# geometryxyz/mental-poker

Measured on AMD Instinct MI355X. Metric: shuffle proofs/sec (prove+verify), higher is better.
Workload: dtype u32 limbs (256-bit Montgomery: 9x29-bit lazy base field, 8x32 scalar field); 1 GPU; pairs: 52-card deck, m=2 n=26, stark curve, shuffle_and_remask + verify_shuffle; rccl_world=1, fixed_base_window_bits=21, unit_counted=prove+verify pairs, streams=1, aggregate_keys=1, transcript_lanes=1, prover_streams=1, pipeline_depth=0, validated_once=False, full=False

## Files before the change

### mental-poker_amd/csrc/engine_core.hpp

```cpp
#pragma once
#include "engine_base.hpp"
#include "kernels_bucket.hpp"
#include "kernels_canonical.hpp"
#include "kernels_sigma.hpp"
#include "kernels_open.hpp"
#include "kernels_deal.hpp"
#include "kernels_sample.hpp"
#include "kernels_screen.hpp"
#include "serialize_host.hpp"
#include "setup_host.hpp"

namespace mp {

static const uint32_t FCHUNK = 8;
static const uint32_t VCHUNK = 64;
static const uint32_t NORM_CHUNK = 64;
static const uint32_t BUCKET_MIN = 2048;
static const uint32_t BUCKET_MIN_SMALL_BATCH = 512;

struct PhaseDev {
  DevBuf<Term> recode, tables, fterms, vterms, cterms, cterms2, cterms0;
  DevBuf<Job> fjobs, vjobs, cjobs, cjobs2, cjobs0;
  DevBuf<BJob> bjobs;
  DevBuf<Term> bterms;
// ... 270 lines not shown
  Workspace ws;
  bool merged_verify = true;
  void set_merged_verify(bool on) override { merged_verify = on; }
  bool subgroup_check = !Cofactor<C>::ONE;
  void set_subgroup_check(bool on) override { subgroup_check = on && !Cofactor<C>::ONE; }
  void check_subgroup(Workspace& w, uint32_t B, uint32_t first, uint32_t count) {
    if (!subgroup_check || !count) return;
    SubgroupArgs a{w.P.p, w.status.p, w.Bpad, first};
    MP_RUN(k_subgroup_check, C, B, count, a);
  }
  void check_verify_inputs(Workspace& w, uint32_t B, const VerifyLay& l, bool keyed) {
    if (!validated) {
      check_subgroup(w, B, 0, l.pk + (keyed ? 1u : 0u));
      return;
    }
    if (!(validated & MP_VALIDATED_DECKS)) check_subgroup(w, B, l.deck, 2 * N);
    if (!(validated & MP_VALIDATED_SHUFFLED)) check_subgroup(w, B, l.shuf, 2 * N);
    const uint32_t rest = std::max(l.deck, l.shuf) + 2 * N;
    if (!(validated & MP_VALIDATED_PROOFS)) check_subgroup(w, B, rest, l.pk - rest);
    if (keyed) check_subgroup(w, B, l.pk, 1);
  }
  Workspace dws;
  void validate_decks_dev(size_t count, const uint8_t* decks, int32_t* status) override {
    rt::Stream s = ctx->stream;
    const uint32_t B = (uint32_t)count;
    Workspace& w = dws;
    w.fw = G_::FW;
    w.ensure(B, 1, 2 * N, 8, 0, 0, nwin, 4, s, 0);
    rt::dzero(w.status.p, (size_t)w.Bpad * 4, s);
    LoadPointsArgs a{decks, w.P.p, w.status.p, w.Bpad, 2 * N, 0};
    MP_RUN(k_load_points, C, B, 2 * N, a);
    if (!Cofactor<C>::ONE) {
      SubgroupArgs sa{w.P.p, w.status.p, w.Bpad, 0};
      MP_RUN(k_subgroup_check, C, B, 2 * N, sa);
    }
    rt::d2d(status, w.status.p, (size_t)B * 4, s);
    rt::stream_sync(s);
  }
  DevBuf<uint32_t> vflag;
  uint32_t* flag_word(bool vlane, rt::Stream s) {
    if (!vflag.n) vflag.alloc(2, s);
    rt::dzero(vflag.p + (vlane ? 1 : 0), 4, s);
    return vflag.p + (vlane ? 1 : 0);
  }
  bool read_flag(bool vlane) {
    uint32_t flag = 0;
    rt::d2h(&flag, vflag.p + (vlane ? 1 : 0), 4, ctx->stream);
    rt::stream_sync(ctx->stream);
    return flag != 0;
  }
  uint32_t nwin = 0;
  FbGeom fbg{8, 32, 255};
  uint32_t init_seed[8];
  DevBuf<uint8_t> io_a, io_b, io_c, io_d, io_e, io_f;
  DevBuf<int32_t> io_status;

  static bool wire_point_host(const uint8_t* p, Aff<C>& out) {
    alignas(8) uint8_t tmp[G_::PB];
    memcpy(tmp, p, G_::PB);
    return wire_to_aff<C>(tmp, out);
  }

  void build_plans(PlanSet* set, bool keyed) {
    rt::Stream s = ctx->stream;
    for (int k = 0; k < N_PLANS; ++k) {
      PlanSet& q = set[k];
      const PlanParams& pp = pprm[k];
      const uint32_t bmin = (bucket_min && k == 3) ? std::min(bucket_min, BUCKET_MIN_SMALL_BATCH) : bucket_min;
      const uint32_t pbits = bucket_bits_of(4 * N + 11 * m + 9);
      q.pplan = make_prove_plan(m, n, pp.fch, pp.vch, G_::PB, keyed, bmin, bk_windows(R::BITS, pbits), toom_cook && (k == 0 || k == 2 || k == 4), pp.vsp, pbits);
      q.vplan = make_verify_plan(m, n, pp.fch, pp.vch, G_::PB, keyed, bmin, bk_windows(R::BITS, pbits), pp.vsp, pbits);
      q.table_group = pp.grp;
      q.norm_chunk = pp.nch;
      for (int i = 0; i < 6; ++i) q.pph[i].upload(q.pplan.ph[i], s);
      q.vph.upload(q.vplan.ph, s);
      q.vmph.upload(q.vplan.mph, s);
      q.mjobs.upload(q.vplan.mjobs, s);
      q.mpairs.upload(q.vplan.mpairs, s);
      q.draws.upload(q.pplan.draws, s);
      q.lin.upload(q.pplan.lin, s);
      q.lin_src.upload(q.pplan.lin_src, s);
      q.lin_coef.upload(q.pplan.lin_coef, s);
      q.consts.upload(toom_constants(q.pplan.toom), s);
      q.pwire.upload(q.pplan.wire, s);
      q.vwire.upload(q.vplan.wire, s);
    }
  }
  void ensure_keyed() {
    if (psk_ready) return;
    build_plans(psk, true);
    const ProveLay& l = psk[0].pplan.lay;
    key_d_first = key_t_first = 0;
    for (int k = 0; k < N_PLANS; ++k)
      for (int i = 0; i < 6; ++i) {
        key_d_first = std::max(key_d_first, psk[k].pplan.ph[i].n_dslots);
        key_t_first = std::max(key_t_first, psk[k].pplan.ph[i].n_tslots);
      }
    std::vector<Term> rec, tab;
    for (uint32_t i = 0; i < N; ++i) rec.push_back(Term{l.rho + i, key_d_first + i});
    for (uint32_t w = 0; w < nwin; ++w) tab.push_back(Term{l.kw + w, key_t_first + w});
    key_recode.upload(rec, ctx->stream);
    key_tables.upload(tab, ctx->stream);
    psk_ready = true;
  }

  int init(mp_ctx* c, uint32_t m_, uint32_t n_, const uint8_t* params, const uint8_t* pk, uint32_t fb_bits, const mp_table* fb_from = nullptr) {
// ... 6 lines not shown
    point_bytes = G_::PB;
    if (G_::FW > 8) bucket_split_bits = 11;
    set_latency_batch(std::max<size_t>(40, (size_t)2560 * 52 / N));
    nwin = (uint32_t)vb_windows(R::BITS);
    default_plan_params();
    FixedBases fb{n};
    std::vector<Aff<C>> bases(fb.count());
    bool ok = true;
    Aff<C> G, H, gen, pkp;
    ok &= wire_point_host(params, G);
    for (uint32_t j = 0; j < n; ++j) ok &= wire_point_host(params + G_::PB * (1 + j), bases[fb.ck(j)]);
    ok &= wire_point_host(params + G_::PB * (1 + n), H);
    ok &= wire_point_host(params + G_::PB * (2 + n), gen);
    ok &= wire_point_host(pk, pkp);
    if (!ok) return fail(MP_ERR_BAD_ENCODING, "parameters / shared key: bad point encoding");
    ok = aff_in_subgroup_host<C>(G) && aff_in_subgroup_host<C>(H) && aff_in_subgroup_host<C>(gen) && aff_in_subgroup_host<C>(pkp);
    for (uint32_t j = 0; j < n; ++j) ok = ok && aff_in_subgroup_host<C>(bases[fb.ck(j)]);
    if (!ok) return fail(MP_ERR_BAD_ENCODING, "parameters / shared key: a point is not in the prime-order subgroup");
    bases[fb.H()] = H; bases[fb.G()] = G; bases[fb.pk()] = pkp; bases[fb.gen()] = gen;
    Jac<C> gs = jac_inf<C>();
    for (uint32_t j = 0; j < n; ++j) gs = jac_madd<C>(gs, bases[fb.ck(j)]);
    if (jac_is_inf<C>(gs)) {
      bases[fb.gsum()] = aff_inf<C>();
    } else {
      bases[fb.gsum()] = jac_to_aff_with_zinv<C>(gs, fe_inv<F>(gs.Z));
    }
    for (uint32_t i = 0; i < fb.count(); ++i)
      if (i != fb.gsum() && aff_is_inf<C>(bases[i])) return fail(MP_ERR_BAD_ENCODING, "parameters: a base is the point at infinity");

    rt::Stream s = ctx->stream;
    std::vector<uint32_t> flat(fb.count() * G_::PW);
    for (uint32_t i = 0; i < fb.count(); ++i) {
      fe_pack<F>(bases[i].x, &flat[i * G_::PW]);
      fe_pack<F>(bases[i].y, &flat[i * G_::PW + G_::FW]);
    }
    fbpts.upload(flat, s);
    if (fb_from) {
      if (fb_from->fb_bits != fb_bits || fb_from->n != n || fb_from->point_bytes != point_bytes || fb_from->ctx->device != ctx->device)
        return fail(MP_ERR_INTERNAL, "shared fixed-base tables: geometry or device mismatch");
      FB.borrow(fb_from->fixed_tables());
    } else {
      build_fixed_tables(fb.count());
    }

    build_plans(ps, false);
    {
      Blake2sState st;
      blake2s_init(st);
      uint32_t mblk[16] = {0};
      memcpy(mblk, "Shuffle Proof", 13);
      blake2s_compress(st, mblk, 13, true);
      memcpy(init_seed, st.h, 32);
    }
    rt::stream_sync(s);
    return MP_OK;
  }

  void normalize_flat(const uint32_t* src, uint32_t* dst, uint32_t* scratch, size_t count) {
    if (!count) return;
    const uint32_t ch = cur_norm_chunk;
    NormArgs a{src, dst, scratch, (uint32_t)count, (uint32_t)((count + ch - 1) / ch), ch};
    MP_RUN(k_normalize, C, a.nthreads, 1, a);
  }

  void build_narrow_tables(const uint32_t* pts, uint32_t nb, const FbGeom& gh, uint32_t h2, uint32_t* out) {
    rt::Stream s = ctx->stream;
    DevBuf<uint32_t> WJ, W, EJ, scratch;
    const size_t nwinpts = (size_t)nb * gh.windows, nent = nwinpts * gh.entries;
    WJ.alloc(nwinpts * G_::JW, s);
    W.alloc(nwinpts * G_::PW, s);
    EJ.alloc(nent * G_::JW, s);
    scratch.alloc(nent * G_::FW, s);
    FbWinArgs wa{pts, WJ.p, gh, h2};
    MP_RUN(k_fb_windows, C, nb, 1, wa);
    normalize_flat(WJ.p, W.p, scratch.p, nwinpts);
    FbFillArgs fa{W.p, EJ.p, gh};
    MP_RUN(k_fb_fill, C, (uint32_t)nwinpts, 1, fa);
    normalize_flat(EJ.p, out, scratch.p, nent);
    rt::stream_sync(s);
  }
  void build_fixed_tables(uint32_t nb) {
    rt::Stream s = ctx->stream;
    const uint32_t h = fbg.bits == 8 ? 8u : (fbg.bits + 1u) / 2u, h2 = fbg.bits == 8 ? 8u : fbg.bits - h;
    const FbGeom gh{h, fbg.bits == 8 ? fbg.windows : 2u * fbg.windows, (1u << h) - 1u};
    DevBuf<uint32_t> Th;
    Th.alloc((size_t)nb * gh.windows * gh.entries * G_::PW, s);
    build_narrow_tables(fbpts.p, nb, gh, h2, Th.p);
    if (fbg.bits == h) {
      std::swap(FB.p, Th.p);
      std::swap(FB.n, Th.n);
      return;
    }
    const size_t nentw = (size_t)nb * fbg.windows * fbg.entries;
    if (nentw >= ((size_t)1 << 32)) throw std::runtime_error("fixed-base table too large for one launch: use narrower windows");
    DevBuf<uint32_t> EJw, scratchw;
    EJw.alloc(nentw * G_::JW, s, false);
    scratchw.alloc(nentw * G_::FW, s, false);
    FB.alloc(nentw * G_::PW, s, false);
    FbWidenArgs ww{Th.p, EJw.p, gh, fbg};
    MP_RUN(k_fb_widen, C, (uint32_t)nentw, 1, ww);
    const size_t per = (size_t)1 << 26;
    for (size_t off = 0; off < nentw; off += per) {
      const size_t cnt = std::min(per, nentw - off);
      normalize_flat(EJw.p + off * G_::JW, FB.p + off * G_::PW, scratchw.p + off * G_::FW, cnt);
    }
    rt::stream_sync(s);
// ... 245 lines not shown
      CombineArgs a{w.J.p, w.P.p, ph.cjobs.p, ph.cterms.p, w.Bpad};
      run_combine(a, B, ph.n_c);
    }
    if (ph.n_c2) {
      CombineArgs a{w.J.p, w.P.p, ph.cjobs2.p, ph.cterms2.p, w.Bpad};
      run_combine(a, B, ph.n_c2);
    }
  }
  void run_normalize(PhaseDev& ph, Workspace& w, uint32_t B, uint32_t norm_only, uint32_t norm_skip, uint32_t* scratch) {
    std::vector<std::pair<uint32_t, uint32_t>> ranges;
    for (auto& r : ph.normalize)
      if ((norm_only == NO_SLOT || r.first == norm_only) && r.first != norm_skip) ranges.push_back(r);
    for (size_t i = 0; i < ranges.size();) {
      const size_t nr = std::min<size_t>(NORM_MAX_RANGES, ranges.size() - i);
      size_t last_elem = 0;
      for (size_t k = 0; k < nr; ++k)
        last_elem = std::max(last_elem, ((size_t)ranges[i + k].first + ranges[i + k].second) * w.Bpad);
      if (nr == 1 || last_elem >= ((size_t)1 << 32)) {
        auto& r = ranges[i];
        normalize_flat(w.J.p + j_off<C>(r.first, w.Bpad, 0), w.P.p + p_off<C>(r.first, w.Bpad, 0), scratch, (size_t)r.second * w.Bpad);
        ++i;
        continue;
      }
      NormMultiArgs a{};
      a.J = w.J.p; a.P = w.P.p; a.scratch = scratch;
      a.nr = (uint32_t)nr; a.chunk = cur_norm_chunk;
      uint32_t threads = 0, selem = 0;
      for (size_t k = 0; k < nr; ++k) {
        auto& r = ranges[i + k];
        const uint32_t cnt = r.second * w.Bpad;
        a.first[k] = r.first * w.Bpad;
        a.count[k] = cnt;
        a.tstart[k] = threads;
        a.sstart[k] = selem;
        threads += (cnt + cur_norm_chunk - 1) / cur_norm_chunk;
        selem += cnt;
      }
      a.tstart[nr] = threads;
      MP_RUN(k_normalize_multi, C, threads, 1, a);
      i += nr;
    }
  }

  FsStatementArgs statement_args(Workspace& w, uint32_t p_deck, uint32_t p_shuf, uint32_t p_cA, uint32_t s_x, uint32_t p_pk = NO_SLOT) {
    FsStatementArgs a{};
    a.f = FsDev{w.stage.p, w.seed.p, w.Bpad};
    a.S = w.S.p;
    a.P = w.P.p;
    a.fbpts = fbpts.p;
    memcpy(a.init_seed, init_seed, 32);
    a.m = m; a.n = n; a.N = N;
    a.p_deck = p_deck; a.p_shuf = p_shuf; a.p_cA = p_cA; a.s_x = s_x;
    a.p_pk = p_pk;
    a.W = nullptr;
    a.w_deck = a.w_shuf = NO_SLOT;
    return a;
  }
  FsqGeom fsq_geom(uint32_t B) const {
    uint32_t lpp = 64;
    while (lpp > 4 && (uint64_t)B * lpp > 65536u) lpp >>= 1;
    return FsqGeom{lpp, B};
  }
  static uint32_t fsq_waves(const FsqGeom& g) { return (g.B + 64u / g.lpp - 1) / (64u / g.lpp); }
  bool fs_quad(uint32_t B) const { return fs_lanes == 4 || (fs_lanes == 0 && B <= FSQ_MAX_BATCH); }
  void run_fs_round1(const FsStatementArgs& a, uint32_t B) {
    if (fs_quad(B)) {
      FsqStatementArgs q{a, fsq_geom(B)};
      MP_WAVE_RUN(k_fsq_round1, C, fsq_waves(q.g), 0, q);
    } else {
      MP_RUN(k_fs_round1, C, B, 1, a);
    }
  }
  void run_fs_round(const FsRoundArgs& a, uint32_t B) {
    if (fs_quad(B)) {
      FsqRoundArgs q{a, fsq_geom(B)};
      MP_WAVE_RUN(k_fsq_round, C, fsq_waves(q.g), 0, q);
    } else {
      MP_RUN(k_fs_round, C, B, 1, a);
    }
  }
  void run_verify_fs(const VerifyFsArgs& a, uint32_t B) {
    if (fs_quad(B)) {
      FsqVerifyArgs q{a, fsq_geom(B)};
      MP_WAVE_RUN(k_fsq_verify, C, fsq_waves(q.g), 0, q);
    } else {
      MP_RUN(k_verify_fs, C, B, 1, a);
    }
  }
  uint32_t* wire_words(Workspace& w, uint32_t B, uint32_t decks) {
    const int plan = plan_of(B);
    if (plan != 1 && plan != 3 && plan != 5) return nullptr;
    w.W.alloc((size_t)decks * 2 * N * (G_::PB / 4) * w.Bpad, ctx->stream, false);
    return w.W.p;
  }

  void prove_init(const ProveInitArgs& ia, uint32_t B) {
    if (B <= PROVE_INIT_WAVE_MAX)
      MP_WAVE_RUN(k_prove_init_w, C, B, N, ia);
    else
      MP_RUN(k_prove_init, C, B, 1, ia);
  }
#ifdef MP_EXP_OVERLAP_MAX
  uint32_t overlap_max = MP_EXP_OVERLAP_MAX;
#else
  uint32_t overlap_max = OVERLAP_MAX_BATCH;
#endif
// ... 1915 lines not shown
```

### mental-poker_amd/csrc/hash.hpp

```cpp
#pragma once
#include <cstdint>

#include "field.hpp"

namespace mp {

MP_HD uint32_t rotr32(uint32_t x, int c) { return (x >> c) | (x << (32 - c)); }
MP_HD uint32_t rotl32(uint32_t x, int c) { return (x << c) | (x >> (32 - c)); }

struct Blake2sState {
  uint32_t h[8];
};

MP_HD void blake2s_init(Blake2sState& s) {
  const uint32_t iv[8] = {0x6A09E667u, 0xBB67AE85u, 0x3C6EF372u, 0xA54FF53Au, 0x510E527Fu, 0x9B05688Cu, 0x1F83D9ABu, 0x5BE0CD19u};
#pragma unroll
  for (int i = 0; i < 8; ++i) s.h[i] = iv[i];
  s.h[0] ^= 0x01010020u;
}

#define MP_B2S_G(a, b, c, d, x, y) \
  v[a] = v[a] + v[b] + (x);        \
  v[d] = rotr32(v[d] ^ v[a], 16);  \
  v[c] = v[c] + v[d];              \
// ... 51 lines not shown
  w.stride = stride;
  w.widx = 0;
  w.acc = 0;
  w.nb = 0;
  return w;
}
MP_HD StageWriter stage_begin_at(uint32_t* stage, uint32_t stride, uint32_t b, uint32_t widx) {
  StageWriter w = stage_begin(stage, stride, b);
  w.widx = widx;
  return w;
}
MP_HD void stage_flush(StageWriter& w) {
  if (w.nb) w.base[(size_t)w.widx * w.stride] = (uint32_t)w.acc;
}
MP_HD void stage_word(StageWriter& w, uint32_t x) {
  w.acc |= (uint64_t)x << (8 * w.nb);
  w.base[(size_t)w.widx * w.stride] = (uint32_t)w.acc;
  w.widx++;
  w.acc >>= 32;
}
MP_HD void stage_byte(StageWriter& w, uint32_t x) {
  w.acc |= (uint64_t)(x & 0xFFu) << (8 * w.nb);
  w.nb++;
  if (w.nb == 4) {
    w.base[(size_t)w.widx * w.stride] = (uint32_t)w.acc;
    w.widx++;
    w.acc = 0;
    w.nb = 0;
  }
}
MP_HD uint32_t stage_len(const StageWriter& w) { return w.widx * 4u + w.nb; }

MP_HD void blake2s_staged(StageWriter& w, uint32_t out[8]) {
  const uint32_t len = stage_len(w);
  if (w.nb) w.base[(size_t)w.widx * w.stride] = (uint32_t)w.acc;
  const uint32_t nwords = (len + 3u) / 4u;
  Blake2sState s;
  blake2s_init(s);
  uint32_t nblocks = (len + 63u) / 64u;
  if (nblocks == 0) nblocks = 1;
  for (uint32_t blk = 0; blk < nblocks; ++blk) {
    uint32_t m[16];
#pragma unroll
    for (int i = 0; i < 16; ++i) {
      uint32_t wi = blk * 16u + i;
      m[i] = wi < nwords ? w.base[(size_t)wi * w.stride] : 0u;
    }
    const bool last = blk + 1 == nblocks;
    const uint64_t t = last ? (uint64_t)len : (uint64_t)(blk + 1) * 64u;
    blake2s_compress(s, m, t, last);
  }
#pragma unroll
  for (int i = 0; i < 8; ++i) out[i] = s.h[i];
}

struct B2sBlock {
  uint32_t w[16];
};
struct B2sSeed {
  uint32_t s[8];
};
MP_HD uint32_t sel4(uint32_t j, uint32_t w0, uint32_t w1, uint32_t w2, uint32_t w3) {
  const uint32_t lo = (j & 1u) ? w1 : w0, hi = (j & 1u) ? w3 : w2;
  return (j & 2u) ? hi : lo;
}
#define MP_B2Q_HALF(x, y)                                                             \
  wv.lanes([&](uint32_t l) {                                                          \
    const uint32_t j = l & 3u;                                                        \
    const B2sBlock& q = m[l];                                                         \
    uint32_t a = va[l], b = vb[l], c = vc[l], d = vd[l];                              \
    a = a + b + (x);                                                                  \
    d = rotr32(d ^ a, 16);                                                            \
    c = c + d;                                                                        \
    b = rotr32(b ^ c, 12);                                                            \
    a = a + b + (y);                                                                  \
    d = rotr32(d ^ a, 8);                                                             \
    c = c + d;                                                                        \
    b = rotr32(b ^ c, 7);                                                             \
    va[l] = a; vb[l] = b; vc[l] = c; vd[l] = d;                                       \
  });
#define MP_B2Q_ROUND(s0, s1, s2, s3, s4, s5, s6, s7, s8, s9, s10, s11, s12, s13, s14, s15)                                   \
  MP_B2Q_HALF(sel4(j, q.w[s0], q.w[s2], q.w[s4], q.w[s6]), sel4(j, q.w[s1], q.w[s3], q.w[s5], q.w[s7]))                     \
  wv.template quad_rot<1>(vb); wv.template quad_rot<2>(vc); wv.template quad_rot<3>(vd);                                    \
  MP_B2Q_HALF(sel4(j, q.w[s8], q.w[s10], q.w[s12], q.w[s14]), sel4(j, q.w[s9], q.w[s11], q.w[s13], q.w[s15]))               \
  wv.template quad_rot<3>(vb); wv.template quad_rot<2>(vc); wv.template quad_rot<1>(vd);
template <class W>
MP_HD void blake2s_compress_quad(W& wv, PerLane<uint32_t>& ha, PerLane<uint32_t>& hb, const PerLane<B2sBlock>& m, uint64_t t, bool last) {
  PerLane<uint32_t> va, vb, vc, vd;
  wv.lanes([&](uint32_t l) {
    const uint32_t j = l & 3u;
    va[l] = ha[l];
    vb[l] = hb[l];
    vc[l] = sel4(j, 0x6A09E667u, 0xBB67AE85u, 0x3C6EF372u, 0xA54FF53Au);
    vd[l] = sel4(j, 0x510E527Fu ^ (uint32_t)t, 0x9B05688Cu ^ (uint32_t)(t >> 32), last ? ~0x1F83D9ABu : 0x1F83D9ABu, 0x5BE0CD19u);
  });
  MP_B2Q_ROUND(0, 1, 2, 3, 4, 5, 6, 7, 8, 9, 10, 11, 12, 13, 14, 15)
  MP_B2Q_ROUND(14, 10, 4, 8, 9, 15, 13, 6, 1, 12, 0, 2, 11, 7, 5, 3)
  MP_B2Q_ROUND(11, 8, 12, 0, 5, 2, 15, 13, 10, 14, 3, 6, 7, 1, 9, 4)
  MP_B2Q_ROUND(7, 9, 3, 1, 13, 12, 11, 14, 2, 6, 5, 10, 4, 0, 15, 8)
  MP_B2Q_ROUND(9, 0, 5, 7, 2, 4, 10, 15, 14, 1, 11, 12, 6, 8, 3, 13)
  MP_B2Q_ROUND(2, 12, 6, 10, 0, 11, 8, 3, 4, 13, 7, 5, 15, 14, 1, 9)
  MP_B2Q_ROUND(12, 5, 1, 15, 14, 13, 4, 10, 0, 7, 6, 3, 9, 2, 8, 11)
  MP_B2Q_ROUND(13, 11, 7, 14, 12, 1, 3, 9, 5, 0, 15, 4, 8, 6, 2, 10)
  MP_B2Q_ROUND(6, 15, 14, 9, 11, 3, 0, 8, 12, 2, 13, 7, 1, 4, 10, 5)
  MP_B2Q_ROUND(10, 2, 8, 4, 7, 6, 1, 5, 15, 11, 9, 14, 3, 12, 13, 0)
  wv.lanes([&](uint32_t l) {
// ... 126 lines not shown
```

### mental-poker_amd/csrc/kernels_proto.hpp

```cpp
#pragma once
#include "hash.hpp"
#include "kernels_msm.hpp"

namespace mp {

enum : int32_t { ST_OK = 0, ST_BAD_ENCODING = -1, ST_BAD_PERMUTATION = -2 };

MP_HD void status_fail(int32_t* status, uint32_t b, int32_t code) {
  status[b] = code;
}

template <class F>
MP_HD bool wire_to_fe(const uint8_t* p, Fe<F>& out) {
  uint32_t k[F::NW];
  const uint32_t* q = reinterpret_cast<const uint32_t*>(p);
#pragma unroll
  for (int i = 0; i < F::NW; ++i) k[i] = q[i];
  const bool ok = fe_canonical_in_range<F>(k);
  out = fe_from_canonical<F>(k);
  return ok;
}
template <class F>
MP_HD void fe_to_wire(const Fe<F>& a, uint8_t* p) {
  uint32_t k[F::NW];
// ... 234 lines not shown
  wv.lanes([&](uint32_t lane) {
    if (lane != 0) return;
    st_fe<R>(a.S + s_off(l.zt + l.m + 1, a.Bpad, b), fe_zero<R>());
    st_fe<R>(a.S + s_off(l.meb + l.m, a.Bpad, b), fe_zero<R>());
    st_fe<R>(a.S + s_off(l.mes + l.m, a.Bpad, b), fe_zero<R>());
    st_fe<R>(a.S + s_off(l.svdelta + l.n - 1, a.Bpad, b), fe_zero<R>());
  });
}
MP_WAVE_KERNEL(k_prove_init_w, ProveInitArgs, body_prove_init_w)

struct FsDev {
  uint32_t* stage;
  uint32_t* seed;
  uint32_t Bpad;
};
template <class C>
MP_HD void fs_put_point(StageWriter& w, const Aff<C>& p) {
  typedef typename C::FqP F;
  constexpr int FW = F::NW;
  uint32_t k[FW];
  if (aff_is_inf<C>(p)) {
    for (int i = 0; i < FW; ++i) stage_word(w, 0);
    stage_word(w, 1);
    for (int i = 1; i < FW; ++i) stage_word(w, 0);
    stage_byte(w, 1);
    return;
  }
  fe_to_canonical<F>(p.x, k);
#pragma unroll
  for (int i = 0; i < FW; ++i) stage_word(w, k[i]);
  fe_to_canonical<F>(p.y, k);
#pragma unroll
  for (int i = 0; i < FW; ++i) stage_word(w, k[i]);
  stage_byte(w, 0);
}
template <class C>
MP_HD void fs_put_wire_point(StageWriter& w, const uint32_t* W, uint32_t slot, uint32_t Bpad, uint32_t b) {
  constexpr int FW = C::FqP::NW, WW = 2 * FW;
  uint32_t k[WW], nz = 0;
  ld_words<WW>(W + ((size_t)slot * Bpad + b) * WW, k);
#pragma unroll
  for (int i = 0; i < WW; ++i) nz |= k[i];
  if (nz == 0) {
    for (int i = 0; i < FW; ++i) stage_word(w, 0);
    stage_word(w, 1);
    for (int i = 1; i < FW; ++i) stage_word(w, 0);
    stage_byte(w, 1);
    return;
  }
#pragma unroll
  for (int i = 0; i < WW; ++i) stage_word(w, k[i]);
  stage_byte(w, 0);
}
MP_HD void fs_load_seed(const FsDev& f, uint32_t b, uint32_t seed[8]) {
#pragma unroll
  for (int i = 0; i < 8; ++i) seed[i] = f.seed[(size_t)i * f.Bpad + b];
}
MP_HD void fs_store_seed(const FsDev& f, uint32_t b, const uint32_t seed[8]) {
#pragma unroll
  for (int i = 0; i < 8; ++i) f.seed[(size_t)i * f.Bpad + b] = seed[i];
}
MP_HD void fs_finish_absorb(StageWriter& w, uint32_t seed[8]) {
#pragma unroll
  for (int i = 0; i < 8; ++i) stage_word(w, seed[i]);
  blake2s_staged(w, seed);
}
template <class C>
MP_HD void fs_absorb_points(const FsDev& f, const uint32_t* P, uint32_t b, uint32_t seed[8], uint32_t first, uint32_t count) {
  StageWriter w = stage_begin(f.stage, f.Bpad, b);
  for (uint32_t i = 0; i < count; ++i) fs_put_point<C>(w, ld_aff<C>(P + p_off<C>(first + i, f.Bpad, b)));
  fs_finish_absorb(w, seed);
}
template <class C>
MP_HD void fs_challenges(const uint32_t seed[8], uint32_t* S, uint32_t Bpad, uint32_t b, uint32_t slot0, uint32_t slot1) {
  typedef typename C::FrP R;
  FrStream st;
  frstream_init(st, seed);
  st_fe<R>(S + s_off(slot0, Bpad, b), frstream_next<R>(st));
  if (slot1 != NO_SLOT) st_fe<R>(S + s_off(slot1, Bpad, b), frstream_next<R>(st));
}

struct FsStatementArgs {
  FsDev f;
  uint32_t* S;
  const uint32_t* P;
  const uint32_t* fbpts;
  uint32_t init_seed[8];
  uint32_t m, n, N;
  uint32_t p_deck, p_shuf, p_cA, s_x;
  uint32_t p_pk;
  const uint32_t* W;
  uint32_t w_deck, w_shuf;
};
MP_HD uint32_t fs_statement_points(const FsStatementArgs& a) { return 4 + a.n + 4 * a.N; }
template <class C>
MP_HD void fs_put_statement_point(StageWriter& w, const FsStatementArgs& a, uint32_t b, uint32_t i) {
  const FixedBases fb{a.n};
  const uint32_t nfix = 4 + a.n;
  if (i < nfix) {
    if (i == 1 && a.p_pk != NO_SLOT) {
      fs_put_point<C>(w, ld_aff<C>(a.P + p_off<C>(a.p_pk, a.f.Bpad, b)));
      return;
    }
    const uint32_t base = i == 0 ? fb.G() : i == 1 ? fb.pk() : i == 2 ? fb.gen() : i == nfix - 1 ? fb.H() : fb.ck(i - 3);
    fs_put_point<C>(w, ld_aff<C>(a.fbpts + (size_t)base * Geo<C>::PW));
    return;
  }
  i -= nfix;
  const bool second = i >= 2 * a.N;
  if (second) i -= 2 * a.N;
  const uint32_t wslot = second ? a.w_shuf : a.w_deck;
  if (a.W && wslot != NO_SLOT)
    fs_put_wire_point<C>(w, a.W, wslot + i, a.f.Bpad, b);
  else
    fs_put_point<C>(w, ld_aff<C>(a.P + p_off<C>((second ? a.p_shuf : a.p_deck) + i, a.f.Bpad, b)));
}
template <class C>
MP_HD void fs_statement_and_x(const FsStatementArgs& a, uint32_t b, uint32_t seed[8]) {
#pragma unroll
  for (int i = 0; i < 8; ++i) seed[i] = a.init_seed[i];
  StageWriter w = stage_begin(a.f.stage, a.f.Bpad, b);
  const uint32_t npts = fs_statement_points(a);
  for (uint32_t i = 0; i < npts; ++i) fs_put_statement_point<C>(w, a, b, i);
  stage_word(w, a.m); stage_word(w, 0); stage_word(w, a.n); stage_word(w, 0);
  fs_finish_absorb(w, seed);
  fs_absorb_points<C>(a.f, a.P, b, seed, a.p_cA, a.m);
  fs_challenges<C>(seed, a.S, a.f.Bpad, b, a.s_x, NO_SLOT);
}
template <class C>
MP_HD void body_fs_round1(const FsStatementArgs& a, uint32_t b, uint32_t y) {
  uint32_t seed[8];
  fs_statement_and_x<C>(a, b, seed);
  fs_store_seed(a.f, b, seed);
}
MP_KERNEL(k_fs_round1, FsStatementArgs, body_fs_round1)

struct FsStep {
  uint32_t first, count;
  uint32_t first2, count2;
  uint32_t slot0, slot1;
};
struct FsRoundArgs {
  FsDev f;
  uint32_t* S;
  uint32_t* P;
  FsStep step[4];
  uint32_t nsteps;
  uint32_t copy_from, copy_to;
};
template <class C>
MP_HD void fs_run_steps(const FsRoundArgs& a, uint32_t b, uint32_t seed[8]) {
  for (uint32_t s = 0; s < a.nsteps; ++s) {
    const FsStep st = a.step[s];
    StageWriter w = stage_begin(a.f.stage, a.f.Bpad, b);
    for (uint32_t i = 0; i < st.count; ++i) fs_put_point<C>(w, ld_aff<C>(a.P + p_off<C>(st.first + i, a.f.Bpad, b)));
    for (uint32_t i = 0; i < st.count2; ++i) fs_put_point<C>(w, ld_aff<C>(a.P + p_off<C>(st.first2 + i, a.f.Bpad, b)));
    fs_finish_absorb(w, seed);
    if (st.slot0 != NO_SLOT) fs_challenges<C>(seed, a.S, a.f.Bpad, b, st.slot0, st.slot1);
  }
}
template <class C>
MP_HD void body_fs_round(const FsRoundArgs& a, uint32_t b, uint32_t y) {
  if (a.copy_from != NO_SLOT)
    st_aff<C>(a.P + p_off<C>(a.copy_to, a.f.Bpad, b), ld_aff<C>(a.P + p_off<C>(a.copy_from, a.f.Bpad, b)));
  uint32_t seed[8];
  fs_load_seed(a.f, b, seed);
  fs_run_steps<C>(a, b, seed);
  fs_store_seed(a.f, b, seed);
}
MP_KERNEL(k_fs_round, FsRoundArgs, body_fs_round)

struct ProveScalArgs {
  uint32_t* S;
  const uint32_t* perm;
  ProveLay l;
  uint32_t Bpad;
  const LinJob* lin;
  const uint32_t* lin_src;
  uint32_t n_lin;
  uint32_t d_parts;
};
#define MP_LD(slot) ld_fe<R>(a.S + s_off((slot), a.Bpad, b))
#define MP_ST(slot, val) st_fe<R>(a.S + s_off((slot), a.Bpad, b), (val))

template <class R>
MP_HD Fe<R> fe_pow_small(const Fe<R>& x, uint32_t e) {
  int top = 31;
  while (!((e >> top) & 1u)) --top;
  Fe<R> acc = x;
  for (int i = top - 1; i >= 0; --i) {
    acc = fe_sqr<R>(acc);
    if ((e >> i) & 1u) acc = fe_mul<R>(acc, x);
  }
  return acc;
}
template <class C>
MP_HD void body_prove_scal1(const ProveScalArgs& a, uint32_t b, uint32_t y) {
  typedef typename C::FrP R;
  const ProveLay& l = a.l;
  uint32_t pi = a.perm[(size_t)b * l.N + y];
  if (pi >= l.N) pi = 0;
  const Fe<R> bi = fe_pow_small<R>(MP_LD(l.x), pi + 1);
  MP_ST(l.b + y, bi);
  MP_ST(l.tmp + y, fe_mul<R>(MP_LD(l.rho + y), bi));
}
MP_KERNEL(k_prove_scal1, ProveScalArgs, body_prove_scal1)
template <class C>
MP_HD void body_prove_scal1b(const ProveScalArgs& a, uint32_t b, uint32_t y) {
  typedef typename C::FrP R;
  const ProveLay& l = a.l;
// ... 223 lines not shown
      MP_ST(l.svat + j, fe_add<R>(fe_mul<R>(x, MP_LD(l.bp + (m - 1) * n + j)), MP_LD(l.svd + j)));
      MP_ST(l.svbt + j, fe_add<R>(fe_mul<R>(x, MP_LD(l.svbp + j)), MP_LD(l.svdelta + j)));
    }
    {
      const Fe<R> x = MP_LD(l.mx);
      Fe<R> ab = MP_LD(l.b + (m - 1) * n + j);
      for (uint32_t i = m - 1; i >= 1; --i) ab = fe_add<R>(fe_mul<R>(ab, x), MP_LD(l.b + (i - 1) * n + j));
      MP_ST(l.meabar + j, fe_add<R>(fe_mul<R>(ab, x), MP_LD(l.mea0 + j)));
    }
    return;
  }
  if (y_ == n) {
    const Fe<R> x = MP_LD(l.zx);
    Fe<R> rb = fe_zero<R>(), sbar = fe_zero<R>(), tb = fe_zero<R>();
    for (uint32_t i = m - 1; i >= 1; --i) rb = fe_mul<R>(fe_add<R>(rb, MP_LD(l.t + i)), x);
    for (uint32_t j = 0; j < m; ++j) sbar = fe_mul<R>(fe_add<R>(sbar, MP_LD(l.zs + j)), x);
    for (uint32_t k = 2 * m + 1; k-- > 0;) tb = fe_add<R>(fe_mul<R>(tb, x), MP_LD(l.zt + k));
    MP_ST(l.zrbar, fe_add<R>(rb, MP_LD(l.zr0)));
    MP_ST(l.zsbar, fe_add<R>(sbar, MP_LD(l.zsm)));
    MP_ST(l.ztbar, tb);
    return;
  }
  if (y_ == n + 1) {
    const Fe<R> x = MP_LD(l.svx);
    MP_ST(l.svrt, fe_add<R>(fe_mul<R>(x, MP_LD(l.sb)), MP_LD(l.svrd)));
    MP_ST(l.svst, fe_add<R>(fe_mul<R>(x, MP_LD(l.svsx)), MP_LD(l.svs1)));
    return;
  }
  {
    const Fe<R> x = MP_LD(l.mx);
    Fe<R> rb = fe_zero<R>(), bb = fe_zero<R>(), sbar = fe_zero<R>(), tb = fe_zero<R>();
    for (uint32_t i = m; i >= 1; --i) rb = fe_mul<R>(fe_add<R>(rb, MP_LD(l.s + i - 1)), x);
    for (uint32_t k = 2 * m; k-- > 0;) {
      bb = fe_add<R>(fe_mul<R>(bb, x), MP_LD(l.meb + k));
      sbar = fe_add<R>(fe_mul<R>(sbar, x), MP_LD(l.mes + k));
      tb = fe_add<R>(fe_mul<R>(tb, x), MP_LD(l.metau + k));
    }
    MP_ST(l.merbar, fe_add<R>(rb, MP_LD(l.mer0)));
    MP_ST(l.mebbar, bb);
    MP_ST(l.mesbar, sbar);
    MP_ST(l.metaubar, tb);
  }
}
MP_KERNEL(k_prove_scal4, ProveScalArgs, body_prove_scal4)

struct VerifyFsArgs {
  FsStatementArgs st;
  VerifyLay l;
  uint32_t merge;
};
template <class C>
MP_HD void fs_merge_weights(const FsDev& f, uint32_t* S, const VerifyLay& l, uint32_t b, uint32_t seed[8]) {
  typedef typename C::FrP R;
  StageWriter w = stage_begin(f.stage, f.Bpad, b);
  for (uint32_t i = 0; i < 5 * l.n + 9; ++i) {
    uint32_t k[8];
    fe_to_canonical<R>(ld_fe<R>(S + s_off(l.zabar + i, f.Bpad, b)), k);
#pragma unroll
    for (int t = 0; t < 8; ++t) stage_word(w, k[t]);
  }
  fs_finish_absorb(w, seed);
  FrStream st;
  frstream_init(st, seed);
  for (uint32_t k = 0; k < (uint32_t)VC_COUNT; ++k) st_fe<R>(S + s_off(l.mr + k, f.Bpad, b), frstream_next<R>(st));
#pragma unroll
  for (int t = 0; t < 8; ++t) f.seed[(size_t)t * f.Bpad + b] = seed[t];
}
template <class C>
MP_HD void body_verify_fs(const VerifyFsArgs& a, uint32_t b, uint32_t y) {
  const VerifyLay& l = a.l;
  const uint32_t m = l.m;
  uint32_t seed[8];
  fs_statement_and_x<C>(a.st, b, seed);
  const FsDev& f = a.st.f;
  uint32_t* S = a.st.S;
  const uint32_t* P = a.st.P;
  fs_absorb_points<C>(f, P, b, seed, l.cB, m);
  fs_challenges<C>(seed, S, f.Bpad, b, l.y, l.z);
  fs_absorb_points<C>(f, P, b, seed, l.cb, 1);
  fs_absorb_points<C>(f, P, b, seed, l.hB, m);
  fs_challenges<C>(seed, S, f.Bpad, b, l.hx, l.hy);
  fs_absorb_points<C>(f, P, b, seed, l.zcA0, 2 + 2 * m + 1);
  fs_challenges<C>(seed, S, f.Bpad, b, l.zx, NO_SLOT);
  fs_absorb_points<C>(f, P, b, seed, l.svcd, 3);
  fs_challenges<C>(seed, S, f.Bpad, b, l.svx, NO_SLOT);
  fs_absorb_points<C>(f, P, b, seed, l.mecA0, 1 + 2 * m + 4 * m);
  fs_challenges<C>(seed, S, f.Bpad, b, l.mx, NO_SLOT);
  if (a.merge) fs_merge_weights<C>(f, S, l, b, seed);
}
MP_KERNEL(k_verify_fs, VerifyFsArgs, body_verify_fs)

struct FsqGeom {
  uint32_t lpp, B;
};
struct FsqLane {
  uint32_t b, sub;
  bool live;
};
MP_HD FsqLane fsq_lane(const FsqGeom& g, uint32_t wid, uint32_t l) {
  FsqLane q;
  const uint32_t b = wid * (64u / g.lpp) + l / g.lpp;
  q.live = b < g.B;
  q.b = q.live ? b : g.B - 1;
  q.sub = l & (g.lpp - 1u);
  return q;
}
template <class C, class W, class PutPoint, class PutTail>
MP_HD void fsq_absorb(W& wv, const FsDev& f, const FsqGeom& g, uint32_t wid, uint32_t npts, PutPoint put_point, uint32_t tail_words,
                      PutTail tail, PerLane<B2sSeed>& seed) {
  constexpr uint32_t GW = 8 * C::FqP::NW + 1;
  const uint32_t ngroups = npts / 4;
  PerLane<const uint32_t*> base;
  wv.lanes([&](uint32_t l) {
    const FsqLane q = fsq_lane(g, wid, l);
    base[l] = f.stage + q.b;
    if (!q.live) return;
    for (uint32_t gi = q.sub; gi < ngroups; gi += g.lpp) {
      StageWriter w = stage_begin_at(f.stage, f.Bpad, q.b, gi * GW);
      for (uint32_t k = 0; k < 4; ++k) put_point(w, q.b, 4 * gi + k);
    }
    if (q.sub == (ngroups & 3u)) {
      StageWriter w = stage_begin_at(f.stage, f.Bpad, q.b, ngroups * GW);
      for (uint32_t i = 4 * ngroups; i < npts; ++i) put_point(w, q.b, i);
      tail(w, q.b);
#pragma unroll
      for (int i = 0; i < 8; ++i) stage_word(w, seed[l].s[i]);
      stage_flush(w);
    }
  });
  wv.sync_global();
  blake2s_staged_quad(wv, base, f.Bpad, npts * GW + 4 * tail_words + 32, seed);
  wv.sync_global();
}
template <class C, class W>
MP_HD void fsq_absorb_points(W& wv, const FsDev& f, const FsqGeom& g, uint32_t wid, const uint32_t* P, uint32_t first, uint32_t count,
                             uint32_t first2, uint32_t count2, PerLane<B2sSeed>& seed) {
  fsq_absorb<C>(wv, f, g, wid, count + count2,
                [&](StageWriter& w, uint32_t b, uint32_t i) {
                  fs_put_point<C>(w, ld_aff<C>(P + p_off<C>(i < count ? first + i : first2 + (i - count), f.Bpad, b)));
                },
// ... 486 lines not shown
```

### mental-poker_amd/csrc/kernels_sigma.hpp

```cpp
#pragma once
#include "kernels_proto.hpp"

namespace mp {

struct SigmaLay {
  uint32_t nb;
  uint32_t x, r, c, z, negc, minus_one;
  uint32_t g, a, A, chk;
};
MP_HD SigmaLay make_sigma_lay(uint32_t nb) {
  SigmaLay l;
  l.nb = nb;
  l.x = 0; l.r = 1; l.c = 2; l.z = 3; l.negc = 4; l.minus_one = 5;
  l.g = 0; l.a = nb; l.A = 2 * nb; l.chk = 3 * nb;
  return l;
}

struct SigmaInitArgs {
  uint32_t* S;
  const uint8_t* seeds;
  SigmaLay l;
  uint32_t Bpad;
  FsDev f;
  const uint32_t* P;
  const uint8_t* fs_init;
};
template <class C>
MP_HD void body_sigma_init(const SigmaInitArgs& a, uint32_t b, uint32_t y) {
  typedef typename C::FrP R;
  uint32_t key[8];
  const uint32_t* sw = reinterpret_cast<const uint32_t*>(a.seeds + (size_t)b * 32);
#pragma unroll
  for (int i = 0; i < 8; ++i) key[i] = sw[i];
  {
    StageWriter w = stage_begin(a.f.stage, a.f.Bpad, b);
    uint32_t k[8];
    fe_to_canonical<R>(ld_fe<R>(a.S + s_off(a.l.x, a.Bpad, b)), k);
#pragma unroll
    for (int i = 0; i < 8; ++i) stage_word(w, k[i]);
    const uint32_t* fw = reinterpret_cast<const uint32_t*>(a.fs_init + (size_t)b * 32);
#pragma unroll
    for (int i = 0; i < 8; ++i) stage_word(w, fw[i]);
    fs_finish_absorb(w, key);
  }
  fs_absorb_points<C>(a.f, a.P, b, key, a.l.g, 2 * a.l.nb);
  FrStream st;
  frstream_init(st, key);
  st_fe<R>(a.S + s_off(a.l.r, a.Bpad, b), frstream_next<R>(st));
}
MP_KERNEL(k_sigma_init, SigmaInitArgs, body_sigma_init)

struct SigmaFsArgs {
  FsDev f;
  uint32_t* S;
  const uint32_t* P;
  const uint8_t* fs_init;
  SigmaLay l;
  uint32_t prove;
};
template <class C>
MP_HD void body_sigma_fs(const SigmaFsArgs& a, uint32_t b, uint32_t y) {
  typedef typename C::FrP R;
  const SigmaLay& l = a.l;
  uint32_t seed[8];
  const uint32_t* sw = reinterpret_cast<const uint32_t*>(a.fs_init + (size_t)b * 32);
#pragma unroll
  for (int i = 0; i < 8; ++i) seed[i] = sw[i];
  fs_absorb_points<C>(a.f, a.P, b, seed, 0, 3 * l.nb);
  if (!a.prove) {
#pragma unroll
    for (int i = 0; i < 8; ++i) a.f.seed[(size_t)i * a.f.Bpad + b] = seed[i];
  }
  fs_challenges<C>(seed, a.S, a.f.Bpad, b, l.c, NO_SLOT);
  const Fe<R> c = ld_fe<R>(a.S + s_off(l.c, a.f.Bpad, b));
  if (a.prove) {
    const Fe<R> z = fe_add<R>(ld_fe<R>(a.S + s_off(l.r, a.f.Bpad, b)), fe_mul<R>(c, ld_fe<R>(a.S + s_off(l.x, a.f.Bpad, b))));
    st_fe<R>(a.S + s_off(l.z, a.f.Bpad, b), z);
  } else {
    st_fe<R>(a.S + s_off(l.negc, a.f.Bpad, b), fe_neg<R>(c));
    st_fe<R>(a.S + s_off(l.minus_one, a.f.Bpad, b), fe_neg<R>(fe_one<R>()));
  }
}
MP_KERNEL(k_sigma_fs, SigmaFsArgs, body_sigma_fs)

struct SigmaIoArgs {
  uint8_t* proofs;
  uint32_t* S;
  uint32_t* P;
  int32_t* status;
  SigmaLay l;
  uint32_t Bpad;
};
template <class C>
MP_HD void body_sigma_store(const SigmaIoArgs& a, uint32_t b, uint32_t y) {
  typedef typename C::FrP R;
  uint8_t* dst = a.proofs + (size_t)b * (a.l.nb * Geo<C>::PB + 32);
// ... 46 lines not shown
```

Before: 722,700 proofs/s.

## Stream Fiat-Shamir absorption through register Blake2s instead of staged global buffer

Replaces the staged transcript path, which wrote serialized points to a global stage buffer and then hashed it, with an incremental in-register Blake2s stream that compresses each 64-byte block as it fills. It also precomputes the hash state over the fixed statement prefix (generators, public key, commitment bases) on the host once and resumes from it per proof, skipping re-hashing those points when no per-proof key is supplied. The goal is to cut global memory traffic and redundant hashing in the transcript kernels. The cost is a larger per-thread state (a stream struct passed by value in kernel args) and more complex byte-alignment logic, which could raise register pressure.

```diff
diff --git a/mental-poker_amd/csrc/engine_core.hpp b/mental-poker_amd/csrc/engine_core.hpp
--- a/mental-poker_amd/csrc/engine_core.hpp
+++ b/mental-poker_amd/csrc/engine_core.hpp
@@ -346,6 +346,7 @@
   uint32_t nwin = 0;
   FbGeom fbg{8, 32, 255};
   uint32_t init_seed[8];
+  B2sStream fs_pre;
   DevBuf<uint8_t> io_a, io_b, io_c, io_d, io_e, io_f;
   DevBuf<int32_t> io_status;
 
@@ -458,6 +459,12 @@
       blake2s_compress(st, mblk, 13, true);
       memcpy(init_seed, st.h, 32);
     }
+    b2s_begin(fs_pre);
+    fs_put_point<C>(fs_pre, G);
+    fs_put_point<C>(fs_pre, pkp);
+    fs_put_point<C>(fs_pre, gen);
+    for (uint32_t j = 0; j < n; ++j) fs_put_point<C>(fs_pre, bases[fb.ck(j)]);
+    fs_put_point<C>(fs_pre, H);
     rt::stream_sync(s);
     return MP_OK;
   }
@@ -809,6 +816,8 @@
     a.m = m; a.n = n; a.N = N;
     a.p_deck = p_deck; a.p_shuf = p_shuf; a.p_cA = p_cA; a.s_x = s_x;
     a.p_pk = p_pk;
+    a.pre = fs_pre;
+    a.pre_pts = p_pk == NO_SLOT ? 4 + n : 0;
     a.W = nullptr;
     a.w_deck = a.w_shuf = NO_SLOT;
     return a;
diff --git a/mental-poker_amd/csrc/hash.hpp b/mental-poker_amd/csrc/hash.hpp
--- a/mental-poker_amd/csrc/hash.hpp
+++ b/mental-poker_amd/csrc/hash.hpp
@@ -127,6 +127,106 @@
   }
 #pragma unroll
   for (int i = 0; i < 8; ++i) out[i] = s.h[i];
+}
+
+struct B2sStream {
+  Blake2sState st;
+  uint32_t m[16];
+  uint32_t nw;
+  uint32_t carry;
+  uint32_t nb;
+  uint32_t t;
+};
+MP_HD void b2s_begin(B2sStream& s) {
+  blake2s_init(s.st);
+#pragma unroll
+  for (int i = 0; i < 16; ++i) s.m[i] = 0;
+  s.nw = s.carry = s.nb = s.t = 0;
+}
+template <int K, int NMAX>
+MP_HD void b2s_place(uint32_t (&m)[16], uint32_t (&r)[NMAX], const uint32_t (&x)[NMAX]) {
+#pragma unroll
+  for (int j = 0; j < NMAX; ++j) {
+    if (K + j < 16)
+      m[(K + j) & 15] = x[j];
+    else
+      r[(K + j - 16) % NMAX] = x[j];
+  }
+}
+template <int NMAX, bool FIN>
+MP_HD void b2s_append(B2sStream& s, const uint32_t (&x)[NMAX], uint32_t cnt, uint32_t len) {
+  static_assert(NMAX <= 16, "one block at the most");
+  uint32_t r[NMAX];
+#pragma unroll
+  for (int i = 0; i < NMAX; ++i) r[i] = 0;
+  switch (s.nw) {
+#define MP_B2S_AT(K) case K: b2s_place<K, NMAX>(s.m, r, x); break;
+    MP_B2S_AT(0) MP_B2S_AT(1) MP_B2S_AT(2) MP_B2S_AT(3) MP_B2S_AT(4) MP_B2S_AT(5) MP_B2S_AT(6) MP_B2S_AT(7) MP_B2S_AT(8)
+    MP_B2S_AT(9) MP_B2S_AT(10) MP_B2S_AT(11) MP_B2S_AT(12) MP_B2S_AT(13) MP_B2S_AT(14) MP_B2S_AT(15) MP_B2S_AT(16)
+#undef MP_B2S_AT
+    default: break;
+  }
+  const uint32_t end = s.nw + cnt;
+  bool more = end > 16u;
+  s.nw = more ? end - 16u : end;
+  if (FIN) {
+    for (;;) {
+      if (!more) {
+#pragma unroll
+        for (int i = 0; i < 16; ++i) s.m[i] = (uint32_t)i < s.nw ? s.m[i] : 0u;
+      }
+      s.t = more ? s.t + 64u : len;
+      blake2s_compress(s.st, s.m, s.t, !more);
+      if (!more) break;
+#pragma unroll
+      for (int i = 0; i < NMAX; ++i) s.m[i] = r[i];
+      more = false;
+    }
+  } else if (more) {
+    s.t += 64u;
+    blake2s_compress(s.st, s.m, s.t, false);
+#pragma unroll
+    for (int i = 0; i < NMAX; ++i) s.m[i] = r[i];
+  }
+}
+template <int N>
+MP_HD uint32_t b2s_phase(const B2sStream& s, const uint32_t (&k)[N], uint32_t* out) {
+  const uint32_t sh = 32u - 8u * s.nb;
+  uint32_t prev = s.carry;
+#pragma unroll
+  for (int i = 0; i < N; ++i) {
+    out[i] = (uint32_t)((((uint64_t)k[i] << 32) | prev) >> sh);
+    prev = k[i];
+  }
+  return prev;
+}
+template <int N>
+MP_HD void b2s_put(B2sStream& s, const uint32_t (&k)[N], bool has_byte, uint32_t byte) {
+  static_assert(N + 1 <= 16, "one block at the most");
+  uint32_t out[N + 1];
+  s.carry = b2s_phase<N>(s, k, out);
+  out[N] = 0;
+  uint32_t cnt = N;
+  if (has_byte) {
+    s.carry = (s.carry >> 8) | (byte << 24);
+    if (++s.nb == 4u) {
+      out[N] = s.carry;
+      cnt = N + 1;
+      s.nb = 0;
+    }
+  }
+  b2s_append<N + 1, false>(s, out, cnt, 0);
+}
+MP_HD void b2s_finish_seed(B2sStream& s, uint32_t seed[8]) {
+  uint32_t k[8], out[9];
+#pragma unroll
+  for (int i = 0; i < 8; ++i) k[i] = seed[i];
+  const uint32_t last = b2s_phase<8>(s, k, out);
+  const uint32_t len = s.t + 4u * s.nw + s.nb + 32u;
+  out[8] = s.nb ? last >> (32u - 8u * s.nb) : 0u;
+  b2s_append<9, true>(s, out, s.nb ? 9u : 8u, len);
+#pragma unroll
+  for (int i = 0; i < 8; ++i) seed[i] = s.st.h[i];
 }
 
 struct B2sBlock {
diff --git a/mental-poker_amd/csrc/kernels_proto.hpp b/mental-poker_amd/csrc/kernels_proto.hpp
--- a/mental-poker_amd/csrc/kernels_proto.hpp
+++ b/mental-poker_amd/csrc/kernels_proto.hpp
@@ -310,6 +310,48 @@
   for (int i = 0; i < WW; ++i) stage_word(w, k[i]);
   stage_byte(w, 0);
 }
+template <class C>
+MP_HD void fs_put_canon(B2sStream& s, const uint32_t* k, bool inf) {
+  constexpr int FW = C::FqP::NW;
+#pragma unroll 1
+  for (int half = 0; half < 2; ++half) {
+    uint32_t h[FW];
+#pragma unroll
+    for (int i = 0; i < FW; ++i) {
+      const uint32_t v = half ? k[FW + i] : k[i];
+      h[i] = inf ? (uint32_t)(half == 1 && i == 0) : v;
+    }
+    b2s_put<FW>(s, h, half == 1, inf ? 1u : 0u);
+  }
+}
+template <class C>
+MP_HD void fs_put_point_at(B2sStream& s, const uint32_t* src, const uint32_t* wire) {
+  typedef typename C::FqP F;
+  constexpr int FW = F::NW, WW = 2 * FW;
+  uint32_t k[WW];
+  bool inf;
+  if (wire) {
+    uint32_t nz = 0;
+    ld_words<WW>(wire, k);
+#pragma unroll
+    for (int i = 0; i < WW; ++i) nz |= k[i];
+    inf = nz == 0;
+  } else {
+    const Aff<C> p = ld_aff<C>(src);
+    inf = aff_is_inf<C>(p);
+    fe_to_canonical<F>(p.x, k);
+    fe_to_canonical<F>(p.y, k + FW);
+  }
+  fs_put_canon<C>(s, k, inf);
+}
+template <class C>
+MP_HD void fs_put_point(B2sStream& s, const Aff<C>& p) {
+  typedef typename C::FqP F;
+  uint32_t k[2 * F::NW];
+  fe_to_canonical<F>(p.x, k);
+  fe_to_canonical<F>(p.y, k + F::NW);
+  fs_put_canon<C>(s, k, aff_is_inf<C>(p));
+}
 MP_HD void fs_load_seed(const FsDev& f, uint32_t b, uint32_t seed[8]) {
 #pragma unroll
   for (int i = 0; i < 8; ++i) seed[i] = f.seed[(size_t)i * f.Bpad + b];
@@ -318,16 +360,14 @@
 #pragma unroll
   for (int i = 0; i < 8; ++i) f.seed[(size_t)i * f.Bpad + b] = seed[i];
 }
-MP_HD void fs_finish_absorb(StageWriter& w, uint32_t seed[8]) {
-#pragma unroll
-  for (int i = 0; i < 8; ++i) stage_word(w, seed[i]);
-  blake2s_staged(w, seed);
-}
-template <class C>
-MP_HD void fs_absorb_points(const FsDev& f, const uint32_t* P, uint32_t b, uint32_t seed[8], uint32_t first, uint32_t count) {
-  StageWriter w = stage_begin(f.stage, f.Bpad, b);
-  for (uint32_t i = 0; i < count; ++i) fs_put_point<C>(w, ld_aff<C>(P + p_off<C>(first + i, f.Bpad, b)));
-  fs_finish_absorb(w, seed);
+template <class C>
+MP_HD void fs_absorb_points(const FsDev& f, const uint32_t* P, uint32_t b, uint32_t seed[8], uint32_t first, uint32_t count,
+                            uint32_t first2 = 0, uint32_t count2 = 0) {
+  B2sStream s;
+  b2s_begin(s);
+  for (uint32_t i = 0; i < count + count2; ++i)
+    fs_put_point_at<C>(s, P + p_off<C>(i < count ? first + i : first2 + (i - count), f.Bpad, b), nullptr);
+  b2s_finish_seed(s, seed);
 }
 template <class C>
 MP_HD void fs_challenges(const uint32_t seed[8], uint32_t* S, uint32_t Bpad, uint32_t b, uint32_t slot0, uint32_t slot1) {
@@ -349,6 +389,8 @@
   uint32_t p_pk;
   const uint32_t* W;
   uint32_t w_deck, w_shuf;
+  B2sStream pre;
+  uint32_t pre_pts;
 };
 MP_HD uint32_t fs_statement_points(const FsStatementArgs& a) { return 4 + a.n + 4 * a.N; }
 template <class C>
@@ -377,11 +419,34 @@
 MP_HD void fs_statement_and_x(const FsStatementArgs& a, uint32_t b, uint32_t seed[8]) {
 #pragma unroll
   for (int i = 0; i < 8; ++i) seed[i] = a.init_seed[i];
-  StageWriter w = stage_begin(a.f.stage, a.f.Bpad, b);
-  const uint32_t npts = fs_statement_points(a);
-  for (uint32_t i = 0; i < npts; ++i) fs_put_statement_point<C>(w, a, b, i);
-  stage_word(w, a.m); stage_word(w, 0); stage_word(w, a.n); stage_word(w, 0);
-  fs_finish_absorb(w, seed);
+  B2sStream s;
+  if (a.pre_pts) {
+    s = a.pre;
+  } else {
+    b2s_begin(s);
+  }
+  const FixedBases fb{a.n};
+  const uint32_t nfix = 4 + a.n, npts = fs_statement_points(a);
+  for (uint32_t i = a.pre_pts; i < npts; ++i) {
+    const uint32_t* src = nullptr;
+    const uint32_t* wire = nullptr;
+    if (i < nfix) {
+      const uint32_t base = i == 0 ? fb.G() : i == 1 ? fb.pk() : i == 2 ? fb.gen() : i == nfix - 1 ? fb.H() : fb.ck(i - 3);
+      src = i == 1 && a.p_pk != NO_SLOT ? a.P + p_off<C>(a.p_pk, a.f.Bpad, b) : a.fbpts + (size_t)base * Geo<C>::PW;
+    } else {
+      const uint32_t j = i - nfix;
+      const bool second = j >= 2 * a.N;
+      const uint32_t k = second ? j - 2 * a.N : j, wslot = second ? a.w_shuf : a.w_deck;
+      if (a.W && wslot != NO_SLOT)
+        wire = a.W + ((size_t)(wslot + k) * a.f.Bpad + b) * (2 * C::FqP::NW);
+      else
+        src = a.P + p_off<C>((second ? a.p_shuf : a.p_deck) + k, a.f.Bpad, b);
+    }
+    fs_put_point_at<C>(s, src, wire);
+  }
+  const uint32_t mn[4] = {a.m, 0, a.n, 0};
+  b2s_put<4>(s, mn, false, 0);
+  b2s_finish_seed(s, seed);
   fs_absorb_points<C>(a.f, a.P, b, seed, a.p_cA, a.m);
   fs_challenges<C>(seed, a.S, a.f.Bpad, b, a.s_x, NO_SLOT);
 }
@@ -410,10 +475,7 @@
 MP_HD void fs_run_steps(const FsRoundArgs& a, uint32_t b, uint32_t seed[8]) {
   for (uint32_t s = 0; s < a.nsteps; ++s) {
     const FsStep st = a.step[s];
-    StageWriter w = stage_begin(a.f.stage, a.f.Bpad, b);
-    for (uint32_t i = 0; i < st.count; ++i) fs_put_point<C>(w, ld_aff<C>(a.P + p_off<C>(st.first + i, a.f.Bpad, b)));
-    for (uint32_t i = 0; i < st.count2; ++i) fs_put_point<C>(w, ld_aff<C>(a.P + p_off<C>(st.first2 + i, a.f.Bpad, b)));
-    fs_finish_absorb(w, seed);
+    fs_absorb_points<C>(a.f, a.P, b, seed, st.first, st.count, st.first2, st.count2);
     if (st.slot0 != NO_SLOT) fs_challenges<C>(seed, a.S, a.f.Bpad, b, st.slot0, st.slot1);
   }
 }
@@ -743,14 +805,14 @@
 template <class C>
 MP_HD void fs_merge_weights(const FsDev& f, uint32_t* S, const VerifyLay& l, uint32_t b, uint32_t seed[8]) {
   typedef typename C::FrP R;
-  StageWriter w = stage_begin(f.stage, f.Bpad, b);
+  B2sStream s;
+  b2s_begin(s);
   for (uint32_t i = 0; i < 5 * l.n + 9; ++i) {
     uint32_t k[8];
     fe_to_canonical<R>(ld_fe<R>(S + s_off(l.zabar + i, f.Bpad, b)), k);
-#pragma unroll
-    for (int t = 0; t < 8; ++t) stage_word(w, k[t]);
-  }
-  fs_finish_absorb(w, seed);
+    b2s_put<8>(s, k, false, 0);
+  }
+  b2s_finish_seed(s, seed);
   FrStream st;
   frstream_init(st, seed);
   for (uint32_t k = 0; k < (uint32_t)VC_COUNT; ++k) st_fe<R>(S + s_off(l.mr + k, f.Bpad, b), frstream_next<R>(st));
@@ -766,17 +828,15 @@
   const FsDev& f = a.st.f;
   uint32_t* S = a.st.S;
   const uint32_t* P = a.st.P;
-  fs_absorb_points<C>(f, P, b, seed, l.cB, m);
-  fs_challenges<C>(seed, S, f.Bpad, b, l.y, l.z);
-  fs_absorb_points<C>(f, P, b, seed, l.cb, 1);
-  fs_absorb_points<C>(f, P, b, seed, l.hB, m);
-  fs_challenges<C>(seed, S, f.Bpad, b, l.hx, l.hy);
-  fs_absorb_points<C>(f, P, b, seed, l.zcA0, 2 + 2 * m + 1);
-  fs_challenges<C>(seed, S, f.Bpad, b, l.zx, NO_SLOT);
-  fs_absorb_points<C>(f, P, b, seed, l.svcd, 3);
-  fs_challenges<C>(seed, S, f.Bpad, b, l.svx, NO_SLOT);
-  fs_absorb_points<C>(f, P, b, seed, l.mecA0, 1 + 2 * m + 4 * m);
-  fs_challenges<C>(seed, S, f.Bpad, b, l.mx, NO_SLOT);
+#pragma unroll 1
+  for (uint32_t r = 0; r < 6; ++r) {
+    const uint32_t first = r == 0 ? l.cB : r == 1 ? l.cb : r == 2 ? l.hB : r == 3 ? l.zcA0 : r == 4 ? l.svcd : l.mecA0;
+    const uint32_t count = r == 0 ? m : r == 1 ? 1 : r == 2 ? m : r == 3 ? 2 + 2 * m + 1 : r == 4 ? 3 : 1 + 2 * m + 4 * m;
+    const uint32_t c0 = r == 0 ? l.y : r == 1 ? NO_SLOT : r == 2 ? l.hx : r == 3 ? l.zx : r == 4 ? l.svx : l.mx;
+    const uint32_t c1 = r == 0 ? l.z : r == 2 ? l.hy : NO_SLOT;
+    fs_absorb_points<C>(f, P, b, seed, first, count);
+    if (c0 != NO_SLOT) fs_challenges<C>(seed, S, f.Bpad, b, c0, c1);
+  }
   if (a.merge) fs_merge_weights<C>(f, S, l, b, seed);
 }
 MP_KERNEL(k_verify_fs, VerifyFsArgs, body_verify_fs)
diff --git a/mental-poker_amd/csrc/kernels_sigma.hpp b/mental-poker_amd/csrc/kernels_sigma.hpp
--- a/mental-poker_amd/csrc/kernels_sigma.hpp
+++ b/mental-poker_amd/csrc/kernels_sigma.hpp
@@ -33,15 +33,16 @@
 #pragma unroll
   for (int i = 0; i < 8; ++i) key[i] = sw[i];
   {
-    StageWriter w = stage_begin(a.f.stage, a.f.Bpad, b);
+    B2sStream s;
+    b2s_begin(s);
     uint32_t k[8];
     fe_to_canonical<R>(ld_fe<R>(a.S + s_off(a.l.x, a.Bpad, b)), k);
-#pragma unroll
-    for (int i = 0; i < 8; ++i) stage_word(w, k[i]);
+    b2s_put<8>(s, k, false, 0);
     const uint32_t* fw = reinterpret_cast<const uint32_t*>(a.fs_init + (size_t)b * 32);
 #pragma unroll
-    for (int i = 0; i < 8; ++i) stage_word(w, fw[i]);
-    fs_finish_absorb(w, key);
+    for (int i = 0; i < 8; ++i) k[i] = fw[i];
+    b2s_put<8>(s, k, false, 0);
+    b2s_finish_seed(s, key);
   }
   fs_absorb_points<C>(a.f, a.P, b, key, a.l.g, 2 * a.l.nb);
   FrStream st;
```

Result: no change. 726,900 proofs/s, median of 6 (+0.6%).
